# jscanvic/Scale-Equivariant-Imaging

Measured on AMD Instinct MI355X. Metric: training images/sec (256x256 crops), proposed-loss deblur, higher is better.
Workload: dtype bf16; 1 GPU; BASELINE configs[1]: deblurring Gaussian_R2 noise=5, proposed loss (SURE + scale-EI), 256x256 pairs cropped to 48 in Loss.forward, ConvolutionalModel hidden=32 scales=5; parameters=645063043, batch_per_gpu=32, global_batch=32, parallelism=dp1

## Files before the change

### include/sei_hip.h

```cpp
#ifndef SEI_HIP_H
#define SEI_HIP_H

#include <stddef.h>
#include <stdint.h>

#ifdef __cplusplus
extern "C" {
#endif

#define SEI_OK 0
#define SEI_ERR_BAD_ARG 10001
#define SEI_ERR_TOO_LARGE 10002


#define SEI_ABI_VERSION 12
int sei_abi_version(void);
int sei_build_target(char *name, int n);

int sei_event_create(void **event);
int sei_event_destroy(void *event);
int sei_event_record_external(void *event, void *stream);
int sei_stream_wait_event(void *stream, void *event);

int sei_graph_node_counts(void *graph, int *kernel_nodes, int *all_nodes);
// ... 51 lines not shown
int sei_conv3x3_bwd_weight(const float *x, const float *gy, float *gw, float *gb, int B, int H, int W,
                           int Cin, int Cout, int nchw_x, int nchw_gy, void *stream);
size_t sei_conv3x3_bwd_weight_parts_count(int B, int H, int W, int Cin, int Cout, int nchw_x, int nchw_gy);
int sei_conv3x3_bwd_weight_parts(const float *x, const float *gy, float *part, int B, int H, int W, int Cin, int Cout,
                                 int nchw_x, int nchw_gy, void *stream);

int sei_dwconv7_fwd(const float *x, const float *w, const float *bias, const float *res,
                    float res_scale, float *y, int B, int H, int W, int C, int flip, void *stream);
size_t sei_dwconv7_bwd_weight_workspace(int B, int H, int W, int C);
int sei_dwconv7_bwd_weight(const float *x, const float *gy, float *gw, float *gbias, int B, int H,
                           int W, int C, float *work, size_t work_floats, void *stream);
int sei_dwconv7_fwd_ex(const float *x, const float *w, const float *bias, const float *res,
                       float res_scale, float *y, int B, int H, int W, int C, int flip, int seg, void *stream);
size_t sei_dwconv7_bwd_weight_workspace_ex(int B, int H, int W, int C, int seg);
int sei_dwconv7_bwd_weight_ex(const float *x, const float *gy, float *gw, float *gbias, int B, int H,
                              int W, int C, float *work, size_t work_floats, int seg, void *stream);
int sei_dwconv7_ln_fwd(const float *x, const float *w, const float *bias, const float *gamma, const float *beta,
                       float *h1, void *h2, int out16, float *mean, float *rstd, int B, int H, int W, int C,
                       float eps, void *stream);
int sei_dwconv7_ln_fwd_ex(const float *x, const float *w, const float *bias, const float *gamma, const float *beta,
                          float *h1, void *h2, int out16, float *mean, float *rstd, int B, int H, int W, int C,
                          float eps, int fuse, void *stream);
size_t sei_dwconv7_ln_fwd_launches(int B, int H, int W, int C);

int sei_ln_fwd(const float *x, const float *gamma, const float *beta, float *y, float *mean,
               float *rstd, size_t rows, int C, float eps, void *stream);
size_t sei_ln_bwd_workspace(size_t rows, int C);
size_t sei_ln_bwd_part_offset(size_t rows, int C);
size_t sei_ln_bwd_part_count(size_t rows, int C);
int sei_ln_bwd(const float *x, const float *gamma, const float *mean, const float *rstd,
               const float *gy, float *gx, float *ggamma, float *gbeta, size_t rows, int C,
               float *work, size_t work_floats, void *stream);
int sei_ln_bwd_res(const float *x, const float *gamma, const float *mean, const float *rstd,
                   const float *gy, const float *res, float *gx, float *ggamma, float *gbeta, size_t rows, int C,
                   float *work, size_t work_floats, void *stream);

#define SEI_FOLD_SPLIT 0
#define SEI_FOLD_DWCONV7 1
#define SEI_FOLD_MAX_JOBS 48
typedef struct SeiFoldJob {
    float *a, *b, *c;
    int ncol, split, kind, nseg;
    const float *part[3];
    int groups[3];
    int reserved;
} SeiFoldJob;
// ... 229 lines not shown
```

### scale-equivariant-imaging_amd/_native.py

```python
import ctypes
import os

import torch

_HERE = os.path.dirname(os.path.abspath(__file__))
LIB_PATH = os.environ.get("SEI_HIP_LIBRARY") or os.path.join(_HERE, "libsei_hip.so")

SEI_REDUCE_BLOCKS = 256

_c = ctypes
_P, _I, _F, _Z, _L = _c.c_void_p, _c.c_int, _c.c_float, _c.c_size_t, _c.c_longlong

SIGNATURES = {
    "sei_abi_version": [],
    "sei_event_create": [_P],
    "sei_event_destroy": [_P],
    "sei_event_record_external": [_P, _P],
    "sei_stream_wait_event": [_P, _P],
    "sei_graph_node_counts": [_P, _P, _P],
    "sei_build_target": [_c.c_char_p, _I],
    "sei_blur_sep_circ": [_P, _P, _P, _P, _I, _I, _I, _I, _I, _I, _P],
    "sei_blur_dense_circ": [_P, _P, _P, _I, _I, _I, _I, _I, _I, _P],
    "sei_resample_sepband": [_P, _P, _I, _I, _I, _I, _I, _P, _P, _I, _I, _P, _P, _I, _I, _P],
    "sei_scale_params": [_P, _P, _P, _I, _I, _P, _P, _P],
# ... 4 lines not shown
    "sei_axpy": [_P, _P, _F, _P, _Z, _P],
    "sei_stack_axpy": [_P, _P, _F, _P, _Z, _P],
    "sei_proposed_draws": [_c.c_ulonglong, _c.c_ulonglong, _P, _I, _I, _I, _I, _I, _P, _I, _P, _P, _P, _P],
    "sei_crop_window": [_P, _P, _I, _I, _I, _I, _I, _I, _P],
    "sei_concat2_f32": [_P, _Z, _P, _Z, _P, _P],
    "sei_scale_dev_f32": [_P, _P, _P, _Z, _P],
    "sei_add_scalars": [_P, _P, _P, _P],
    "sei_zero_ranges": [_P, _P, _I, _P],
    "sei_sure_terms": [_P, _P, _P, _P, _I, _I, _I, _I, _I, _F, _F, _F, _P, _P, _P, _P, _P],
    "sei_mse_terms": [_P, _P, _Z, _F, _P, _P, _P, _P],
    "sei_sure_loss": [_P, _P, _P, _P, _I, _I, _I, _I, _I, _F, _F, _F, _F, _P, _P, _P, _P, _P],
    "sei_mse_loss": [_P, _P, _Z, _F, _F, _P, _P, _P, _P],
    "sei_luma_sqerr": [_P, _P, _Z, _P, _P, _P],
    "sei_ssim_luma": [_P, _P, _I, _I, _I, _P, _P, _P],
    "sei_conv3x3_fwd": [_P, _P, _P, _P, _P, _I, _I, _I, _I, _I, _I, _I, _I, _P],
    "sei_conv3x3_bwd_weight": [_P, _P, _P, _P, _I, _I, _I, _I, _I, _I, _I, _P],
    "sei_conv3x3_bwd_weight_parts": [_P, _P, _P, _I, _I, _I, _I, _I, _I, _I, _P],
    "sei_dwconv7_fwd": [_P, _P, _P, _P, _F, _P, _I, _I, _I, _I, _I, _P],
    "sei_dwconv7_bwd_weight": [_P, _P, _P, _P, _I, _I, _I, _I, _P, _Z, _P],
    "sei_dwconv7_fwd_ex": [_P, _P, _P, _P, _F, _P, _I, _I, _I, _I, _I, _I, _P],
    "sei_dwconv7_bwd_weight_ex": [_P, _P, _P, _P, _I, _I, _I, _I, _P, _Z, _I, _P],
    "sei_dwconv7_ln_fwd": [_P, _P, _P, _P, _P, _P, _P, _I, _P, _P, _I, _I, _I, _I, _F, _P],
    "sei_dwconv7_ln_fwd_ex": [_P, _P, _P, _P, _P, _P, _P, _I, _P, _P, _I, _I, _I, _I, _F, _I, _P],
    "sei_ln_fwd": [_P, _P, _P, _P, _P, _P, _Z, _I, _F, _P],
    "sei_ln_bwd": [_P, _P, _P, _P, _P, _P, _P, _P, _Z, _I, _P, _Z, _P],
    "sei_ln_bwd_res": [_P, _P, _P, _P, _P, _P, _P, _P, _P, _Z, _I, _P, _Z, _P],
    "sei_gemm_f32": [_P, _P, _P, _I, _I, _I, _I, _I, _I, _P, _P, _P, _P, _P],
    "sei_gemm_f32_ex": [_P, _P, _P, _I, _I, _I, _I, _I, _I, _P, _P, _P, _P, _I, _L, _L, _L, _I, _P],
    "sei_gemm_bf16_ex": [_P, _P, _P, _I, _I, _I, _I, _I, _I, _P, _P, _P, _P, _I, _L, _L, _L, _I, _P],
    "sei_gemm_bf16_mixed": [_P, _I, _P, _I, _P, _I, _I, _I, _I, _I, _I, _P, _P, _P, _P, _I, _L, _L, _L, _I, _P],
    "sei_cast_bf16": [_P, _P, _Z, _P],
    "sei_weight_shadow_bf16": [_P, _P, _P, _I, _I, _P],
    "sei_ln_fwd_bf16": [_P, _P, _P, _P, _P, _P, _Z, _I, _F, _P],
    "sei_colsum_bf16": [_P, _P, _Z, _I, _P],
    "sei_split_bf16x2": [_P, _P, _Z, _P],
    "sei_split_bf16x3": [_P, _P, _Z, _I, _P],
    "sei_gelu_f32": [_P, _P, _Z, _P],
    "sei_mul_dgelu_f32": [_P, _P, _Z, _P],
    "sei_cast_transpose_bf16": [_P, _I, _P, _P, _I, _I, _I, _P, _P],
    "sei_cast_bf16_colsum_weighted": [_P, _P, _P, _P, _I, _I, _P],
    "sei_cast_bf16_colsum_parts": [_P, _P, _P, _P, _I, _I, _P],
    "sei_gemm_bf16nt": [_P, _I, _I, _P, _I, _I, _P, _P, _I, _I, _I, _I, _P, _P, _P, _P, _P],
    "sei_gemm_bf16nt_colsum": [_P, _I, _I, _P, _I, _I, _P, _I, _I, _I, _I, _P, _P, _P],
    "sei_gemm_bf16nt_ws": [_P, _I, _I, _P, _I, _I, _P, _P, _I, _I, _I, _I, _P, _P, _P, _P, _P, _P, _Z, _I, _I, _I, _P],
    "sei_fold_many": [_P, _I, _P],
    "sei_transpose_bf16_many": [_P, _I, _P],
# ... 64 lines not shown
DWSTREAM_MAX_JOBS = 64


class FoldJob(_c.Structure):
    _fields_ = [("a", _P), ("b", _P), ("c", _P), ("ncol", _I), ("split", _I), ("kind", _I), ("nseg", _I),
                ("part", _P * 3), ("groups", _I * 3), ("reserved", _I)]


FOLD_SPLIT, FOLD_DWCONV7, FOLD_MAX_JOBS = 0, 1, 48


class TransposeJob(_c.Structure):
    _fields_ = [("src", _P), ("dst", _P), ("R", _I), ("C", _I)]


TRANSPOSE_MAX_JOBS = 16


SIZE_QUERIES = {
    "sei_proposed_draws_max_numel": [],
    "sei_ssim_luma_work_floats": [_I, _I, _I],
    "sei_dwconv7_bwd_weight_workspace": [_I, _I, _I, _I],
    "sei_dwconv7_bwd_weight_workspace_ex": [_I, _I, _I, _I, _I],
    "sei_ln_bwd_workspace": [_Z, _I],
    "sei_dwconv7_ln_fwd_launches": [_I, _I, _I, _I],
    "sei_sepmap2_bf16_eligible": [_I, _I, _I, _I, _I, _I],
    "sei_sepmap2_bf16_pack_elems": [_I, _I, _I, _I],
    "sei_sepmap2_big_eligible": [_I, _I, _I, _I, _I, _I],
    "sei_sepmap2_big_pack_elems": [_I, _I, _I, _I],
    "sei_sepmap2_big_work_elems": [_I, _I, _I, _I, _I, _I],
    "sei_swin_partials_floats": [_I],
    "sei_tokgrad_bf16_eligible": [_I, _I, _I, _I, _L, _L],
    "sei_dwstream_bf16_eligible": [_I, _I, _I, _I, _L, _L],
    "sei_mlp_fused_eligible": [_L, _I],
    "sei_rowgemm_bf16_eligible": [_L, _I, _I, _I, _I],
    "sei_rowgemm_lnbwd_bf16_eligible": [_L, _I, _I],
    "sei_rowgemm_lnbwd_work_floats": [_I],
    "sei_ln_bwd_part_offset": [_Z, _I],
    "sei_ln_bwd_part_count": [_Z, _I],
    "sei_rowgemm_dgelu_bf16_eligible": [_L, _I, _I],
    "sei_rowgemm_ln_bf16_eligible": [_L, _I, _I],
    "sei_gemm_bf16nt_plan": [_I, _I, _I, _I, _I, _I, _I, _I],
    "sei_gemm_bf16nt_plan_ws": [_I, _I, _I, _I, _I, _I, _I, _I, _Z],
    "sei_conv3x3_bwd_weight_parts_count": [_I, _I, _I, _I, _I, _I, _I],
    "sei_sepmap2_small_eligible": [_I, _I, _I, _I, _I, _I],
    "sei_cast_bf16_colsum_parts_count": [_I, _I],
# ... 152 lines not shown
```

### scale-equivariant-imaging_amd/models/_ops.py

```python
import os

import torch

import _native as N
from . import _mats

EPI_NONE, EPI_BIAS, EPI_BIAS_GELU, EPI_BIAS_RES, EPI_MUL_DGELU, EPI_ACCUM, EPI_BIAS_ROWSCALE = range(7)
LN_EPS = 1e-6


def grad_of(p):
    if p.grad is None:
        view = getattr(p, "_sei_grad_view", None)
        if view is None or view.shape != p.shape or view.device != p.device:
            view = torch.zeros_like(p, memory_format=torch.contiguous_format)
        else:
            view.zero_()
        p.grad = view
    return p.grad


_ARENA = None


# ... 347 lines not shown
    M = B * H * W
    h1 = _alloc((B, H, W, C), torch.float32, x.device)
    h2 = _alloc((M, C), torch.bfloat16 if out16 else torch.float32, x.device)
    mean = _alloc((M,), torch.float32, x.device)
    rstd = _alloc((M,), torch.float32, x.device)
    args = (x.data_ptr(), w.data_ptr(), N.ptr(bias), gamma.data_ptr(), beta.data_ptr(), h1.data_ptr(), h2.data_ptr(),
            int(out16), mean.data_ptr(), rstd.data_ptr(), B, H, W, C, LN_EPS)
    if fuse:
        N.call("sei_dwconv7_ln_fwd_ex", *args, int(fuse))
    else:
        N.call("sei_dwconv7_ln_fwd", *args)
    return h1, h2, mean, rstd


def dwconv7_weight_grad(x, gy, gw, gb, seg=0):
    B, H, W, C = x.shape
    need = N.lib().sei_dwconv7_bwd_weight_workspace_ex(B, H, W, C, int(seg))
    work = torch.empty(need, dtype=torch.float32, device=x.device)
    deferred = need > 0 and defer_fold(gw, gb, None, 50 * C, C, N.FOLD_DWCONV7, work, 0, need // (50 * C))
    leaf_call(gw, "sei_dwconv7_bwd_weight_ex", x.data_ptr(), gy.data_ptr(), None if deferred else gw.data_ptr(),
              None if deferred else N.ptr(gb), B, H, W, C, work.data_ptr(), need, int(seg), keep=(x, gy, work))


def sepmap2(x, mats, Ho, Wo):
    B, Hi, Wi, C = x.shape
    y = _alloc((B, Ho, Wo, C), torch.float32, x.device)
    work = torch.empty(2 * B * Hi * Wo * C, dtype=torch.float32, device=x.device)
    RW, LH = (mats[4], mats[5]) if len(mats) >= 6 else _mats.pack_for_kernel(mats[:4], x.device)
    N.call("sei_sepmap2_packed", x.data_ptr(), y.data_ptr(), B, Hi, Wi, Ho, Wo, C, RW.data_ptr(), LH.data_ptr(),
           work.data_ptr(), work.numel())
    return y


_SEPMAP_MFMA = __import__("os").environ.get("SEI_SEPMAP_F32") != "1"
_SEPMAP_SMALL = __import__("os").environ.get("SEI_NO_SEPMAP_SMALL") != "1"


def sepmap2_16(x, mats, Ho, Wo, out16=False):
    B, Hi, Wi, C = x.shape
    if _SEPMAP_SMALL and x.is_cuda and N.lib().sei_sepmap2_small_eligible(B, Hi, Wi, Ho, Wo, C):
        y = _alloc((B, Ho, Wo, C), torch.bfloat16 if out16 else torch.float32, x.device)
        L1, R1, L2, R2 = mats[:4]
        N.call("sei_sepmap2_small", x.data_ptr(), y.data_ptr(), int(out16), B, Hi, Wi, Ho, Wo, C, L1.data_ptr(),
               R1.data_ptr(), L2.data_ptr(), R2.data_ptr())
        return y
    small = _SEPMAP_MFMA and x.is_cuda and max(Hi, Wi, Ho, Wo) <= 64 and N.lib().sei_sepmap2_bf16_eligible(B, Hi, Wi, Ho, Wo, C)
# ... 16 lines not shown


def _packed16(mats, big=False):
    L1, R1, L2, R2 = mats[:4]
    key = (L1.data_ptr(), R1.data_ptr(), L2.data_ptr(), R2.data_ptr(), tuple(L1.shape), tuple(R1.shape), big)
    hit = _PACKED16.get(key)
    if hit is None:
        (Ho, Hi), (Wo, Wi) = L1.shape, R1.shape
        kind = "sei_sepmap2_big" if big else "sei_sepmap2_bf16"
        out = torch.empty(getattr(N.lib(), kind + "_pack_elems")(Hi, Wi, Ho, Wo), dtype=torch.int16, device=L1.device)
        N.call(kind + "_pack", L1.data_ptr(), R1.data_ptr(), L2.data_ptr(), R2.data_ptr(), out.data_ptr(), Hi, Wi,
               Ho, Wo)
        hit = _PACKED16[key] = (out, L1, R1, L2, R2)
    return hit[0]


def _nhwc(x):
    N.check_tensor(x, "activation")
    if x.dim() != 4:
        raise ValueError("expected an NHWC activation (B, H, W, C)")
    return x


class ConvBlockFn(torch.autograd.Function):
    @staticmethod
    def forward(ctx, x, w1, b1, gamma, beta, w2, b2, w3, b3, twice):
        _no_joint_form()
        ctx.dtype = get_compute_dtype()
        x = _nhwc(x)
        B, H, W, C = x.shape
        M = B * H * W
        h1, h2, mean, rstd = dwconv7_ln(x, w1, b1, gamma, beta, out16=False)
        h4 = torch.empty((M, 4 * C), dtype=torch.float32, device=x.device)
        h3 = gemm(h2, w2, M, 4 * C, C, 0, 1, EPI_BIAS_GELU, bias=b2, D2=h4)
        out = gemm(h4, w3, M, C, 4 * C, 0, 1, EPI_BIAS_RES, bias=b3, R1=x, R2=x if twice else None)
        ctx.save_for_backward(x, h1, mean, rstd, h2, h3, h4)
        ctx.params = (w1, b1, gamma, beta, w2, b2, w3, b3)
        ctx.twice = twice
        return out.view(B, H, W, C)

    @_in_forward_mode
    def backward(ctx, go):
        x, h1, mean, rstd, h2, h3, h4 = ctx.saved_tensors
        w1, b1, gamma, beta, w2, b2, w3, b3 = ctx.params
        B, H, W, C = x.shape
        M = B * H * W
        go = go.contiguous()
        go2 = go.view(M, C)
        colsum_into(grad_of(b3), go2)
        gemm(go2, h4, C, 4 * C, M, 1, 0, EPI_ACCUM, out=grad_of(w3).view(C, 4 * C))
        gh3 = gemm(go2, w3, M, 4 * C, C, 0, 0, EPI_MUL_DGELU, R1=h3)
        colsum_into(grad_of(b2), gh3)
        gemm(gh3, h2, 4 * C, C, M, 1, 0, EPI_ACCUM, out=grad_of(w2).view(4 * C, C))
        gh2 = gemm(gh3, w2, M, C, 4 * C, 0, 0, EPI_NONE)
        gh1 = layer_norm_bwd(h1.view(M, C), gamma, mean, rstd, gh2, grad_of(gamma), grad_of(beta))
        gh1 = gh1.view(B, H, W, C)
        dwconv7_weight_grad(x, gh1, grad_of(w1), grad_of(b1))
        gx = None
        if ctx.needs_input_grad[0]:
            gx = dwconv7(gh1, w1, None, flip=True, res=go, res_scale=2.0 if ctx.twice else 1.0)
        return (gx,) + (None,) * 9


class DownsampleFn(torch.autograd.Function):

    @staticmethod
    def forward(ctx, x, gamma, beta, w, b, rate, with_skip=False):
        _no_joint_form()
        ctx.dtype = get_compute_dtype()
        ctx.set_materialize_grads(False)
        x = _nhwc(x)
        B, H, W, C = x.shape
        M, Co = B * H * W, w.shape[0]
        h, mean, rstd = layer_norm(x.view(M, C), gamma, beta)
        fwd, bwd = _mats.resample_matrices("down", H, W, rate, x.device)
        Ho, Wo = fwd[0].shape[0], fwd[1].shape[0]
        u = sepmap2(h.view(B, H, W, C), fwd, Ho, Wo)
        Mo = B * Ho * Wo
        s = _mats.constant_response("down", H, W, rate, x.device, B)
        out = gemm(u.view(Mo, C), w, Mo, Co, C, 0, 1, EPI_BIAS_ROWSCALE, bias=b, R1=s)
        ctx.save_for_backward(x, mean, rstd, u, s)
        ctx.params, ctx.mats_t, ctx.hw = (gamma, beta, w, b), bwd, (H, W, Ho, Wo)
        out = out.view(B, Ho, Wo, Co)
        return (out, x) if with_skip else out
# ... 156 lines not shown
    M, Nn = x16.shape
    if leaf:
        leaf_call(acc, "sei_colsum_bf16", x16.data_ptr(), acc.data_ptr(), M, Nn, keep=(x16,))
    else:
        N.call("sei_colsum_bf16", x16.data_ptr(), acc.data_ptr(), M, Nn)


def colsum16_into_inline(acc, x16):
    colsum16_into(acc, x16, leaf=False)


def gemm_mixed(A, Bm, M, Nn, K, ta, tb, epi, out=None, bias=None, R1=None, R2=None, D2=None, allow_splitk=True):
    if out is None:
        out = torch.empty((M, Nn), dtype=torch.float32, device=A.device)
    _gemm_call(2.0 * M * Nn * K, "sei_gemm_bf16_mixed", A.data_ptr(), int(A.dtype == torch.bfloat16), Bm.data_ptr(),
               int(Bm.dtype == torch.bfloat16), out.data_ptr(), M, Nn, K, ta, tb, epi, N.ptr(bias), N.ptr(R1),
               N.ptr(R2), N.ptr(D2), 1, 0, 0, 0, int(allow_splitk))
    return out


CAST_COLSUM_PARTS = os.environ.get("SEI_CAST_COLSUM_ATOMICS") != "1"


def cast16(x2d, colsum_into_=None, row_weight=None):
    R, C = x2d.shape
    x16 = _alloc((R, C), torch.bfloat16, x2d.device)
    if colsum_into_ is not None and CAST_COLSUM_PARTS and C % 4 == 0:
        parts = N.lib().sei_cast_bf16_colsum_parts_count(R, C)
        ms = _state_for(colsum_into_.data_ptr())["milestone"]
        early = ms is not None and min(ms[0]) <= colsum_into_.data_ptr() <= max(ms[0])
        if parts > 0 and not early:
            work = torch.empty(parts * C, dtype=torch.float32, device=x2d.device)
            if defer_fold(colsum_into_, None, None, C, C, N.FOLD_SPLIT, work, 0, parts):
                N.call("sei_cast_bf16_colsum_parts", x2d.data_ptr(), x16.data_ptr(), N.ptr(row_weight), work.data_ptr(), R, C)
                return x16
    if row_weight is not None and colsum_into_ is not None and C % 4 == 0:
        N.call("sei_cast_bf16_colsum_weighted", x2d.data_ptr(), x16.data_ptr(), row_weight.data_ptr(), colsum_into_.data_ptr(),
               R, C)
        return x16
    if row_weight is not None and colsum_into_ is not None:
        colsum_into(colsum_into_, x2d, row_weight=row_weight)
        colsum_into_ = None
    N.call("sei_cast_transpose_bf16", x2d.data_ptr(), 0, x16.data_ptr(), None, R, C, R, N.ptr(colsum_into_))
    return x16


def _fresh_state():
# ... 440 lines not shown
        part = stale[k:k + N.TRANSPOSE_MAX_JOBS]
        outs = [torch.empty((q16.shape[1], q16.shape[0]), dtype=torch.bfloat16, device=q16.device) for _, q16, _ in part]
        jobs = (N.TransposeJob * len(part))(*[N.TransposeJob(q16.data_ptr(), o.data_ptr(), q16.shape[0], q16.shape[1])
                                             for (_, q16, _), o in zip(part, outs)])
        N.call("sei_transpose_bf16_many", jobs, len(part))
        for (q, _, qkey), o in zip(part, outs):
            q._sei_shadow_t = (qkey, o, capturing)
    return p._sei_shadow_t[1]


def _transposed16(w16):
    R, C = w16.shape
    wt = torch.empty((C, R), dtype=torch.bfloat16, device=w16.device)
    N.call("sei_cast_transpose_bf16", w16.data_ptr(), 1, None, wt.data_ptr(), R, C, R, None)
    return wt


class ConvBlockFn16(torch.autograd.Function):

    @staticmethod
    def forward(ctx, x, w1, b1, gamma, beta, w2, b2, w3, b3, twice):
        ctx.dtype = get_compute_dtype()
        x = _nhwc(x)
        B, H, W, C = x.shape
        M = B * H * W
        h1, h2, mean, rstd = dwconv7_ln(x, w1, b1, gamma, beta, out16=True)
        w2_16, w3_16 = shadow(w2), shadow(w3)
        ctx.fused = fused_mlp_ok(M, C)
        _tape(ConvBlockFn16, ctx)
        if ctx.fused:
            out = _alloc((M, C), torch.float32, x.device)
            N.call("sei_mlp_fused_fwd", h2.data_ptr(), w2_16.data_ptr(), b2.data_ptr(), w3_16.data_ptr(), b3.data_ptr(),
                   x.data_ptr(), 2.0 if twice else 1.0, out.data_ptr(), M, C)
            if _GEMM_PROFILE is not None:
                _GEMM_PROFILE.append((4.0 * M * 4 * C * C, "sei_mlp_fused_fwd",
                                      (h2.data_ptr(), w2_16.data_ptr(), b2.data_ptr(), w3_16.data_ptr(), b3.data_ptr(),
                                       x.data_ptr(), 2.0 if twice else 1.0, out.data_ptr(), M, C)))
            ctx.save_for_backward(x, h1, mean, rstd, h2)
            ctx.params = (w1, b1, gamma, beta, w2, b2, w3, b3)
            ctx.twice = twice
            return out.view(B, H, W, C)
        h3 = _alloc((M, 4 * C), torch.float32, x.device)
        h4 = _alloc((M, 4 * C), torch.bfloat16, x.device)
        gemm_nt16(h2, w2_16, M, 4 * C, C, EPI_BIAS_GELU, out32=h3, bias=b2, D2_16=h4)
        out = _alloc((M, C), torch.float32, x.device)
        gemm_nt16(h4, w3_16, M, C, 4 * C, EPI_BIAS_RES, out32=out, bias=b3, R1=x, R2=x if twice else None)
        ctx.save_for_backward(x, h1, mean, rstd, h2, h3, h4)
        ctx.params = (w1, b1, gamma, beta, w2, b2, w3, b3)
        ctx.twice = twice
        return out.view(B, H, W, C)

    @_in_forward_mode
    def backward(ctx, go):
        if ctx.fused:
            return ConvBlockFn16._backward_fused(ctx, go)
        x, h1, mean, rstd, h2, h3, h4 = ctx.saved_tensors
        w1, b1, gamma, beta, w2, b2, w3, b3 = ctx.params
        B, H, W, C = x.shape
        M = B * H * W
        go = go.contiguous()
        go2 = go.view(M, C)
        go16 = cast16(go2, colsum_into_=grad_of(b3))
        gh3 = torch.empty((M, 4 * C), dtype=torch.bfloat16, device=x.device)
        gemm_nt16(go16, shadow(w3), M, 4 * C, C, EPI_MUL_DGELU, out16=gh3, R1=h3, b_rmajor=True, colsum=grad_of(b2))
        weight_grad16(go16, h4, grad_of(w3).view(C, 4 * C))
        gh2 = torch.empty((M, C), dtype=torch.float32, device=x.device)
        gemm_nt16(gh3, shadow(w2), M, C, 4 * C, EPI_NONE, out32=gh2, b_rmajor=True)
        weight_grad16(gh3, h2, grad_of(w2).view(4 * C, C))
        gh1 = layer_norm_bwd(h1.view(M, C), gamma, mean, rstd, gh2, grad_of(gamma), grad_of(beta)).view(B, H, W, C)
        dwconv7_weight_grad(x, gh1, grad_of(w1), grad_of(b1))
        gx = None
        if ctx.needs_input_grad[0]:
            gx = dwconv7(gh1, w1, None, flip=True, res=go, res_scale=2.0 if ctx.twice else 1.0)
        return (gx,) + (None,) * 9


    @staticmethod
    def _backward_fused(ctx, go):
        x, h1, mean, rstd, h2 = ctx.saved_tensors
        w1, b1, gamma, beta, w2, b2, w3, b3 = ctx.params
        B, H, W, C = x.shape
        M = B * H * W
        go = go.contiguous()
        dev = x.device
        w2_16, w3_16 = shadow(w2), shadow(w3)
        gh2 = torch.empty((M, C), dtype=torch.float32, device=dev)
        go16 = torch.empty((M, C), dtype=torch.bfloat16, device=dev)
        h4 = torch.empty((M, 4 * C), dtype=torch.bfloat16, device=dev)
        gh3 = torch.empty((M, 4 * C), dtype=torch.bfloat16, device=dev)
        w3t, w2t = _transposed16_cached(w3, w3_16), _transposed16_cached(w2, w2_16)
        args = (go.data_ptr(), h2.data_ptr(), w2_16.data_ptr(), b2.data_ptr(), w3t.data_ptr(), w2t.data_ptr(),
                gh2.data_ptr(), go16.data_ptr(), h4.data_ptr(), gh3.data_ptr(), M, C)
        N.call("sei_mlp_fused_bwd", *args)
        if _GEMM_PROFILE is not None:
            _GEMM_PROFILE.append((4.0 * M * 4 * C * C, "sei_mlp_fused_bwd", args))
        if DWSTREAM and N.lib().sei_dwstream_bf16_eligible(C, 4 * C, C, 4 * C, M, 0):
            weight_grad16(go16, h4, grad_of(w3).view(C, 4 * C), bias=grad_of(b3))
            weight_grad16(gh3, h2, grad_of(w2).view(4 * C, C), bias=grad_of(b2))
        else:
            colsum_into(grad_of(b3), go.view(M, C))
            colsum16_into(grad_of(b2), gh3)
            weight_grad16(go16, h4, grad_of(w3).view(C, 4 * C))
            weight_grad16(gh3, h2, grad_of(w2).view(4 * C, C))
        gh1 = layer_norm_bwd(h1.view(M, C), gamma, mean, rstd, gh2, grad_of(gamma), grad_of(beta)).view(B, H, W, C)
        dwconv7_weight_grad(x, gh1, grad_of(w1), grad_of(b1))
        gx = None
        if ctx.needs_input_grad[0]:
            gx = dwconv7(gh1, w1, None, flip=True, res=go, res_scale=2.0 if ctx.twice else 1.0)
        return (gx,) + (None,) * 9


class DownsampleFn16(torch.autograd.Function):

    @staticmethod
    def forward(ctx, x, gamma, beta, w, b, rate, with_skip=False):
        ctx.dtype = get_compute_dtype()
        ctx.set_materialize_grads(False)
        x = _nhwc(x)
        B, H, W, C = x.shape
        M, Co = B * H * W, w.shape[0]
        h, mean, rstd = layer_norm(x.view(M, C), gamma, beta)
        fwd, bwd = _mats.resample_matrices("down", H, W, rate, x.device)
        Ho, Wo = fwd[0].shape[0], fwd[1].shape[0]
        u = sepmap2_16(h.view(B, H, W, C), fwd, Ho, Wo, out16=True)
        Mo = B * Ho * Wo
        s = _mats.constant_response("down", H, W, rate, x.device, B)
        u16 = u.view(Mo, C) if u.dtype == torch.bfloat16 else cast16(u.view(Mo, C))
        out = _alloc((Mo, Co), torch.float32, x.device)
        gemm_nt16(u16, shadow(w), Mo, Co, C, EPI_BIAS_ROWSCALE, out32=out, bias=b, R1=s)
        ctx.save_for_backward(x, mean, rstd, u16, s)
        ctx.params, ctx.mats_t, ctx.hw = (gamma, beta, w, b), bwd, (H, W, Ho, Wo)
        ctx.with_skip, ctx.rate = with_skip, rate
        _tape(DownsampleFn16, ctx)
        out = out.view(B, Ho, Wo, Co)
        return (out, x) if with_skip else out

    @_in_forward_mode
    def backward(ctx, go, gskip=None):
        x, mean, rstd, u16, s = ctx.saved_tensors
        gamma, beta, w, b = ctx.params
        B, H, W, C = x.shape
        Ho, Wo = ctx.hw[2], ctx.hw[3]
        M, Mo, Co = B * H * W, B * Ho * Wo, w.shape[0]
        go2 = go.contiguous().view(Mo, Co)
        go16 = cast16(go2, colsum_into_=grad_of(b), row_weight=s)
        gu = torch.empty((Mo, C), dtype=torch.float32, device=x.device)
        gemm_nt16(go16, shadow(w), Mo, C, Co, EPI_NONE, out32=gu, b_rmajor=True)
        weight_grad16(go16, u16, grad_of(w).view(Co, C))
        gh = sepmap2_16(gu.view(B, Ho, Wo, C), ctx.mats_t, H, W).view(M, C)
        res = None if gskip is None else gskip.contiguous().view(M, C)
        gx = layer_norm_bwd(x.view(M, C), gamma, mean, rstd, gh, grad_of(gamma), grad_of(beta), res=res).view(B, H, W, C)
        return (gx if ctx.needs_input_grad[0] else None), None, None, None, None, None, None


class UpsampleFn16(torch.autograd.Function):
    @staticmethod
    def forward(ctx, x, skip, gamma, beta, w, b, rate):
        ctx.dtype = get_compute_dtype()
        x = _nhwc(x)
        B, H, W, C = x.shape
        Co = w.shape[0]
        fwd, bwd = _mats.resample_matrices("up", H, W, rate, x.device)
        Ho, Wo = fwd[0].shape[0], fwd[1].shape[0]
        u = sepmap2_16(x, fwd, Ho, Wo)
        M = B * Ho * Wo
        h, mean, rstd = layer_norm16(u.view(M, C), gamma, beta)
        w16 = shadow(w)
        out = _alloc((M, Co), torch.float32, x.device)
        _tape(UpsampleFn16, ctx)
        if skip is not None:
            skip = _nhwc(skip)
            if tuple(skip.shape) != (B, Ho, Wo, Co):
                raise ValueError("skip connection shape mismatch")
            gemm_nt16(h, w16, M, Co, C, EPI_BIAS_RES, out32=out, bias=b, R1=skip)
        else:
            gemm_nt16(h, w16, M, Co, C, EPI_BIAS, out32=out, bias=b)
        ctx.save_for_backward(u, mean, rstd, h)
        ctx.params, ctx.mats_t, ctx.in_hw = (gamma, beta, w, b), bwd, (H, W)
        return out.view(B, Ho, Wo, Co)

    @_in_forward_mode
    def backward(ctx, go):
        u, mean, rstd, h = ctx.saved_tensors
        gamma, beta, w, b = ctx.params
        B, Ho, Wo, C = u.shape
        M, Co = B * Ho * Wo, w.shape[0]
        go = go.contiguous()
        go2 = go.view(M, Co)
        go16 = cast16(go2, colsum_into_=grad_of(b))
        gh = torch.empty((M, C), dtype=torch.float32, device=u.device)
        gemm_nt16(go16, shadow(w), M, C, Co, EPI_NONE, out32=gh, b_rmajor=True)
        weight_grad16(go16, h, grad_of(w).view(Co, C))
        gu = layer_norm_bwd(u.view(M, C), gamma, mean, rstd, gh, grad_of(gamma), grad_of(beta))
        gx = None
        if ctx.needs_input_grad[0]:
            gx = sepmap2_16(gu.view(B, Ho, Wo, C), ctx.mats_t, *ctx.in_hw)
        gskip = go if ctx.needs_input_grad[1] else None
        return gx, gskip, None, None, None, None, None


class Conv3x3Fn(torch.autograd.Function):
    @staticmethod
    def forward(ctx, x, w, b, res, nchw_in, nchw_out):
        N.check_tensor(x, "conv3x3 input")
        Co, Ci = w.shape[0], w.shape[1]
        if nchw_in:
            B, _, H, W = x.shape
        else:
            B, H, W, _ = x.shape
        y = _alloc((B, Co, H, W) if nchw_out else (B, H, W, Co), torch.float32, x.device)
        _tape(Conv3x3Fn, ctx)
        if res is not None:
# ... 88 lines not shown
```

Before: 2721 images/s.

## Fuse depthwise 7x7 conv backward input and weight gradients into one tiled kernel

Adds a HIP kernel that computes the depthwise 7x7 input gradient and weight/bias gradient in one pass over a shared LDS tile of the output gradient. Global-to-LDS loads are double-buffered. The same kernel can also emit a bf16 copy of the input gradient plus partial column sums, so the next Down/Upsample backward can skip its separate cast16 and colsum pass. This removes repeated reads of gy and x and extra launches per ConvBlock backward, at the cost of a large, register-heavy kernel with one workgroup per CU and more complex fold and side-channel bookkeeping.

Result: no change. 2720 images/s, median of 2 (-0.1%).

```diff
diff --git a/include/sei_hip.h b/include/sei_hip.h
--- a/include/sei_hip.h
+++ b/include/sei_hip.h
@@ -97,6 +97,11 @@
                           float *h1, void *h2, int out16, float *mean, float *rstd, int B, int H, int W, int C,
                           float eps, int fuse, void *stream);
 size_t sei_dwconv7_ln_fwd_launches(int B, int H, int W, int C);
+size_t sei_dwconv7_bwd_pair_workspace(int B, int H, int W, int C);
+size_t sei_dwconv7_bwd_pair_colparts(int B, int H, int W, int C);
+int sei_dwconv7_bwd_pair(const float *x, const float *gy, const float *w, const float *res, float res_scale,
+                         float *gx, uint16_t *gx16, const float *row_weight, float *colpart, float *work,
+                         size_t work_floats, int B, int H, int W, int C, void *stream);
 
 int sei_ln_fwd(const float *x, const float *gamma, const float *beta, float *y, float *mean,
                float *rstd, size_t rows, int C, float eps, void *stream);
diff --git a/scale-equivariant-imaging_amd/_native.py b/scale-equivariant-imaging_amd/_native.py
--- a/scale-equivariant-imaging_amd/_native.py
+++ b/scale-equivariant-imaging_amd/_native.py
@@ -50,6 +50,7 @@
     "sei_dwconv7_bwd_weight_ex": [_P, _P, _P, _P, _I, _I, _I, _I, _P, _Z, _I, _P],
     "sei_dwconv7_ln_fwd": [_P, _P, _P, _P, _P, _P, _P, _I, _P, _P, _I, _I, _I, _I, _F, _P],
     "sei_dwconv7_ln_fwd_ex": [_P, _P, _P, _P, _P, _P, _P, _I, _P, _P, _I, _I, _I, _I, _F, _I, _P],
+    "sei_dwconv7_bwd_pair": [_P, _P, _P, _P, _F, _P, _P, _P, _P, _P, _Z, _I, _I, _I, _I, _P],
     "sei_ln_fwd": [_P, _P, _P, _P, _P, _P, _Z, _I, _F, _P],
     "sei_ln_bwd": [_P, _P, _P, _P, _P, _P, _P, _P, _Z, _I, _P, _Z, _P],
     "sei_ln_bwd_res": [_P, _P, _P, _P, _P, _P, _P, _P, _P, _Z, _I, _P, _Z, _P],
@@ -160,6 +161,8 @@
     "sei_ssim_luma_work_floats": [_I, _I, _I],
     "sei_dwconv7_bwd_weight_workspace": [_I, _I, _I, _I],
     "sei_dwconv7_bwd_weight_workspace_ex": [_I, _I, _I, _I, _I],
+    "sei_dwconv7_bwd_pair_workspace": [_I, _I, _I, _I],
+    "sei_dwconv7_bwd_pair_colparts": [_I, _I, _I, _I],
     "sei_ln_bwd_workspace": [_Z, _I],
     "sei_dwconv7_ln_fwd_launches": [_I, _I, _I, _I],
     "sei_sepmap2_bf16_eligible": [_I, _I, _I, _I, _I, _I],
diff --git a/scale-equivariant-imaging_amd/csrc/dwconv_pair.hip b/scale-equivariant-imaging_amd/csrc/dwconv_pair.hip
--- /dev/null
+++ b/scale-equivariant-imaging_amd/csrc/dwconv_pair.hip
@@ -0,0 +1,375 @@
+#include "sei_common.h"
+
+namespace {
+
+typedef __attribute__((address_space(3))) void lds_void;
+typedef __attribute__((address_space(1))) const void glb_void;
+
+__device__ __attribute__((aligned(16))) float g_pr_zero_chunk[4] = {0.f, 0.f, 0.f, 0.f};
+
+constexpr int PR_THREADS = 256;
+constexpr int PR_CC = 32;
+constexpr int PR_ROWS = PR_THREADS / PR_CC;
+constexpr int PR_MAXK = 10;
+constexpr int PR_WBYTES = PR_CC * 49 * 4;
+constexpr int PR_WPIECES = 7;
+constexpr int PR_SUMS = 52;
+
+__device__ __forceinline__ unsigned short pr_f2bf(float v) {
+    const __bf16 b = (__bf16)v;
+    return __builtin_bit_cast(unsigned short, b);
+}
+
+__device__ __forceinline__ void pr_csum(float &cs, float &comp, float w, float v, bool weighted) {
+    const float p = weighted ? w * v : v;
+    const float y = p - (weighted ? comp - fmaf(w, v, -p) : comp);
+    const float t = cs + y;
+    comp = (t - cs) - y;
+    cs = t;
+}
+
+__device__ __forceinline__ void pr_wait_vmcnt(int n) {
+    switch (n) {
+#define SEI_PR_W(N_) case N_: asm volatile("s_waitcnt vmcnt(" #N_ ")" ::: "memory"); break;
+        SEI_PR_W(1) SEI_PR_W(2) SEI_PR_W(3) SEI_PR_W(4) SEI_PR_W(5) SEI_PR_W(6) SEI_PR_W(7) SEI_PR_W(8)
+        SEI_PR_W(9) SEI_PR_W(10) SEI_PR_W(11) SEI_PR_W(12) SEI_PR_W(13) SEI_PR_W(14) SEI_PR_W(15) SEI_PR_W(16)
+#undef SEI_PR_W
+        default: asm volatile("s_waitcnt vmcnt(0)" ::: "memory"); break;
+    }
+}
+
+constexpr int pr_pieces(int tw) { return ((PR_ROWS + 6) * (tw + 6) + 7) / 8; }
+constexpr int pr_lds_bytes(int tw) { return 2 * pr_pieces(tw) * 1024; }
+static_assert(pr_lds_bytes(12) >= PR_ROWS * PR_SUMS * PR_CC * 4 && pr_pieces(12) * 1024 >= PR_WPIECES * 1024,
+              "the tile buffers also hold the weights (prologue) and the reduction of the sums (epilogue)");
+static_assert(pr_lds_bytes(16) <= 160 * 1024, "one workgroup per CU");
+
+template <int TW>
+__global__ __launch_bounds__(PR_THREADS, 1) void dwconv7_pair_tiled_kernel(
+    const float *__restrict__ x, const float *__restrict__ gy, const float *__restrict__ w,
+    const float *__restrict__ res, float res_scale, float *__restrict__ gx, unsigned short *__restrict__ gx16,
+    const float *__restrict__ row_weight, float *__restrict__ colpart, float *__restrict__ part, int H, int W, int C,
+    int th, int tiles_i, int tiles_j, int ntiles, int tiles_per_block, int npix, int npieces) {
+    constexpr int tw = TW, lw = TW + 6, tile_bytes = pr_pieces(TW) * 1024;
+    __shared__ __attribute__((aligned(16))) char smem[pr_lds_bytes(TW)];
+    const int lane = threadIdx.x & 63, wave = __builtin_amdgcn_readfirstlane(threadIdx.x >> 6);
+    const int cl = threadIdx.x & (PR_CC - 1), tr = threadIdx.x >> 5;
+    const int g = blockIdx.y, c0 = g * PR_CC;
+    const int s0 = blockIdx.x * tiles_per_block, s1 = min(ntiles, s0 + tiles_per_block);
+
+    int pp[PR_MAXK];
+#pragma unroll
+    for (int k = 0; k < PR_MAXK; ++k) {
+        const int pixel = 8 * (wave + 4 * k) + (lane >> 3);
+        const int lr = pixel / lw;
+        pp[k] = pixel < npix ? (lr << 8) | (pixel - lr * lw) : -1;
+    }
+    struct Tile {
+        int b, i0, j0;
+    };
+    auto decode = [&](int s) {
+        Tile t;
+        const int tj = s % tiles_j, rest = s / tiles_j;
+        const int ti = rest % tiles_i;
+        t.b = rest / tiles_i;
+        t.i0 = ti * th;
+        t.j0 = tj * tw;
+        return t;
+    };
+    auto issue_tile = [&](const Tile &t, char *dst) {
+        const float *gb = gy + (size_t)t.b * H * W * C + c0 + 4 * (lane & 7);
+#pragma unroll
+        for (int k = 0; k < PR_MAXK; ++k) {
+            const int q = wave + 4 * k;
+            if (q < npieces) {
+                const int lr = pp[k] >> 8, lc = pp[k] & 255;
+                const int ii = t.i0 - 3 + lr, jj = t.j0 - 3 + lc;
+                const bool ok = pp[k] >= 0 && ii >= 0 && ii < H && jj >= 0 && jj < W;
+                const float *src = ok ? gb + ((size_t)ii * W + jj) * C : g_pr_zero_chunk;
+                __builtin_amdgcn_global_load_lds((glb_void *)src, (lds_void *)(dst + q * 1024), 16, 0, 0);
+            }
+        }
+    };
+    char *const tile0 = smem;
+
+    Tile cur = decode(s0);
+    issue_tile(cur, tile0);
+    {
+        const char *wsrc = reinterpret_cast<const char *>(w + (size_t)c0 * 49);
+#pragma unroll
+        for (int k = 0; k < 2; ++k) {
+            const int p = wave + 4 * k;
+            if (p < PR_WPIECES) {
+                const int off = 1024 * p + 16 * lane;
+                const char *src = off < PR_WBYTES ? wsrc + off : reinterpret_cast<const char *>(g_pr_zero_chunk);
+                __builtin_amdgcn_global_load_lds((glb_void *)src, (lds_void *)(smem + tile_bytes + p * 1024), 16, 0, 0);
+            }
+        }
+    }
+    asm volatile("s_waitcnt vmcnt(0)" ::: "memory");
+    __syncthreads();
+    float wr[49];
+    {
+        const float *wl = reinterpret_cast<const float *>(smem + tile_bytes);
+#pragma unroll
+        for (int t = 0; t < 49; ++t) wr[t] = wl[cl * 49 + 48 - t];
+    }
+    __syncthreads();
+
+    float acc[49];
+#pragma unroll
+    for (int t = 0; t < 49; ++t) acc[t] = 0.f;
+    float acc_b = 0.f, cs = 0.f, cs_comp = 0.f;
+
+    int later = 0;
+    for (int s = s0; s < s1; ++s) {
+        const int par = (s - s0) & 1;
+        const char *tile = tile0 + par * tile_bytes;
+        pr_wait_vmcnt(later);
+        __builtin_amdgcn_s_barrier();
+        asm volatile("" ::: "memory");
+        const int i = cur.i0 + tr;
+        const bool row_ok = tr < th && i < H;
+        const int jn = min(tw, W - cur.j0);
+        const size_t pix0 = ((size_t)cur.b * H + i) * W + cur.j0;
+        const size_t obase = pix0 * C + c0 + cl;
+        float gv[TW], xv[TW];
+        float rw_own = 1.f;
+        if (row_ok) {
+#pragma unroll
+            for (int jl = 0; jl < TW; ++jl) xv[jl] = (jl < jn) ? x[obase + (size_t)jl * C] : 0.f;
+            if (res) {
+#pragma unroll
+                for (int jl = 0; jl < TW; ++jl) gv[jl] = (jl < jn) ? res[obase + (size_t)jl * C] : 0.f;
+            }
+            if (row_weight && cl < jn) rw_own = row_weight[pix0 + cl];
+        }
+        asm volatile("" ::: "memory");
+        Tile nxt = cur;
+        if (s + 1 < s1) {
+            nxt = decode(s + 1);
+            issue_tile(nxt, tile0 + (par ^ 1) * tile_bytes);
+        }
+        asm volatile("" ::: "memory");
+        {
+            const int r0 = 2 * wave;
+            later = (r0 < th && cur.i0 + r0 < H) ? jn : 0;
+        }
+        if (row_ok) {
+            const float *trow = reinterpret_cast<const float *>(tile) + (tr * lw) * PR_CC + cl;
+            constexpr int rs_ = lw * PR_CC;
+            constexpr int RW = 10;
+            const int hw = lane & 32;
+            float ring[7][RW];
+#pragma unroll
+            for (int c = 0; c < 6; ++c)
+#pragma unroll
+                for (int di = 0; di < 7; ++di) ring[di][c % RW] = trow[di * rs_ + c * PR_CC];
+#pragma unroll
+            for (int blk = 0; blk < TW / 4; ++blk) {
+#pragma unroll
+                for (int c = 4 * blk + 6; c < 4 * blk + 10; ++c)
+#pragma unroll
+                    for (int di = 0; di < 7; ++di) ring[di][c % RW] = trow[di * rs_ + c * PR_CC];
+                float a[4] = {0.f, 0.f, 0.f, 0.f};
+#pragma unroll
+                for (int di = 0; di < 7; ++di)
+#pragma unroll
+                    for (int dj = 0; dj < 7; ++dj)
+#pragma unroll
+                        for (int o = 0; o < 4; ++o) {
+                            const float v = ring[di][(4 * blk + o + dj) % RW];
+                            a[o] = fmaf(wr[di * 7 + dj], v, a[o]);
+                            acc[di * 7 + dj] = fmaf(xv[4 * blk + o], v, acc[di * 7 + dj]);
+                        }
+#pragma unroll
+                for (int o = 0; o < 4; ++o) {
+                    const int jl = 4 * blk + o;
+                    if (res) a[o] = fmaf(res_scale, gv[jl], a[o]);
+                    const float rwv = row_weight ? __shfl(rw_own, hw + jl, 64) : 1.f;
+                    if (jl < jn) {
+                        gx[obase + (size_t)jl * C] = a[o];
+                        if (gx16) gx16[obase + (size_t)jl * C] = pr_f2bf(a[o]);
+                        acc_b += ring[3][(jl + 3) % RW];
+                        pr_csum(cs, cs_comp, rwv, a[o], row_weight != nullptr);
+                    }
+                }
+            }
+        }
+        cur = nxt;
+    }
+
+    __syncthreads();
+    float *red = reinterpret_cast<float *>(smem);
+#pragma unroll
+    for (int t = 0; t < 49; ++t) red[(tr * PR_SUMS + 48 - t) * PR_CC + cl] = acc[t];
+    red[(tr * PR_SUMS + 49) * PR_CC + cl] = acc_b;
+    red[(tr * PR_SUMS + 50) * PR_CC + cl] = cs;
+    red[(tr * PR_SUMS + 51) * PR_CC + cl] = cs_comp;
+    __syncthreads();
+    float *out = part + (size_t)blockIdx.x * 50 * C + c0;
+    for (int e = threadIdx.x; e < 51 * PR_CC; e += PR_THREADS) {
+        const int t = e >> 5, c2 = e & 31;
+        if (t < 50) {
+            float sum = 0.f;
+#pragma unroll
+            for (int r = 0; r < PR_ROWS; ++r) sum += red[(r * PR_SUMS + t) * PR_CC + c2];
+            out[(size_t)t * C + c2] = sum;
+        } else if (colpart) {
+            double sum = 0.0;
+#pragma unroll
+            for (int r = 0; r < PR_ROWS; ++r)
+                sum += (double)red[(r * PR_SUMS + 50) * PR_CC + c2] - (double)red[(r * PR_SUMS + 51) * PR_CC + c2];
+            colpart[(size_t)blockIdx.x * C + c0 + c2] = (float)sum;
+        }
+    }
+}
+
+template <int S>
+__global__ __launch_bounds__(PR_THREADS) void dwconv7_pair_whole_kernel(
+    const float *__restrict__ x, const float *__restrict__ gy, const float *__restrict__ w,
+    const float *__restrict__ res, float res_scale, float *__restrict__ gx, unsigned short *__restrict__ gx16,
+    const float *__restrict__ row_weight, float *__restrict__ colpart, float *__restrict__ part, int B, int C,
+    int imgs_per_thread) {
+    __shared__ float wl[PR_THREADS * 49];
+    const int c0 = blockIdx.x * PR_THREADS, c = c0 + threadIdx.x;
+    {
+        const int nw = min(PR_THREADS, C - c0) * 49;
+        for (int e = threadIdx.x; e < nw; e += PR_THREADS) wl[e] = w[(size_t)c0 * 49 + e];
+        __syncthreads();
+    }
+    if (c >= C) return;
+    const int b0 = blockIdx.y * imgs_per_thread, b1 = min(B, b0 + imgs_per_thread);
+    constexpr int LO = (S >= 4) ? 0 : 4 - S, HI = 6 - LO;
+    float wr[49], acc[49];
+#pragma unroll
+    for (int t = 0; t < 49; ++t) {
+        const int di = t / 7, dj = t % 7;
+        const bool used = di >= LO && di <= HI && dj >= LO && dj <= HI;
+        wr[t] = used ? wl[threadIdx.x * 49 + 48 - t] : 0.f;
+        acc[t] = 0.f;
+    }
+    float acc_b = 0.f, cs = 0.f, cs_comp = 0.f;
+    for (int b = b0; b < b1; ++b) {
+        const size_t base = (size_t)b * S * S * C + c;
+        float gi[S][S], xi[S][S];
+#pragma unroll
+        for (int i = 0; i < S; ++i)
+#pragma unroll
+            for (int j = 0; j < S; ++j) {
+                gi[i][j] = gy[base + (size_t)(i * S + j) * C];
+                xi[i][j] = x[base + (size_t)(i * S + j) * C];
+                acc_b += gi[i][j];
+            }
+#pragma unroll
+        for (int i = 0; i < S; ++i)
+#pragma unroll
+            for (int j = 0; j < S; ++j) {
+                float a = 0.f;
+#pragma unroll
+                for (int di = 0; di < 7; ++di)
+#pragma unroll
+                    for (int dj = 0; dj < 7; ++dj) {
+                        const int ii = i + di - 3, jj = j + dj - 3;
+                        if (ii >= 0 && ii < S && jj >= 0 && jj < S) {
+                            a = fmaf(wr[di * 7 + dj], gi[ii][jj], a);
+                            acc[di * 7 + dj] = fmaf(xi[i][j], gi[ii][jj], acc[di * 7 + dj]);
+                        }
+                    }
+                const size_t o = base + (size_t)(i * S + j) * C;
+                if (res) a = fmaf(res_scale, res[o], a);
+                gx[o] = a;
+                if (gx16) gx16[o] = pr_f2bf(a);
+                pr_csum(cs, cs_comp, row_weight ? row_weight[(size_t)b * S * S + i * S + j] : 1.f, a, row_weight != nullptr);
+            }
+    }
+    float *out = part + (size_t)blockIdx.y * 50 * C + c;
+#pragma unroll
+    for (int t = 0; t < 49; ++t) out[(size_t)(48 - t) * C] = acc[t];
+    out[(size_t)49 * C] = acc_b;
+    if (colpart) colpart[(size_t)blockIdx.y * C + c] = cs - cs_comp;
+}
+
+struct PrPlan {
+    int kind;
+    int th, tw, tiles_i, tiles_j, ntiles, tpb, npix, npieces, ipt;
+    unsigned gx, gy;
+    size_t nparts;
+};
+
+inline PrPlan pr_plan(int B, int H, int W, int C) {
+    PrPlan p{};
+    if (B <= 0 || H <= 0 || W <= 0 || C <= 0 || C % PR_CC != 0) return p;
+    if ((size_t)B * H * W * C >= ((size_t)1 << 40)) return p;
+    if ((H == 3 && W == 3) || (H == 6 && W == 6)) {
+        p.gx = (unsigned)sei_ceil_div(C, PR_THREADS);
+        size_t want = (size_t)B * H * W / 64;
+        if (want < 8) want = 8;
+        if (want * p.gx < 256) want = sei_ceil_div(256, p.gx);
+        if (want > (size_t)B) want = B;
+        p.ipt = (int)sei_ceil_div(B, want);
+        p.gy = (unsigned)sei_ceil_div(B, p.ipt);
+        if (p.gy > 65535) return p;
+        p.nparts = p.gy;
+        p.kind = H;
+        return p;
+    }
+    if (H < 8 || W < 8) return p;
+    const int G = C / PR_CC;
+    if (G > 65535) return p;
+    p.th = (H % 8 == 0) ? 8 : ((H % 6 == 0) ? 6 : ((H % 7 == 0) ? 7 : 8));
+    p.tw = (W % 12 == 0) ? 12 : 16;
+    p.tiles_i = (int)sei_ceil_div(H, p.th);
+    p.tiles_j = (int)sei_ceil_div(W, p.tw);
+    const size_t nt = (size_t)B * p.tiles_i * p.tiles_j;
+    if (nt >= ((size_t)1 << 30)) return p;
+    p.ntiles = (int)nt;
+    p.npix = (p.th + 6) * (p.tw + 6);
+    p.npieces = (p.npix + 7) / 8;
+    size_t want = 256 / (size_t)G;
+    if (want < 8) want = 8;
+    p.tpb = (int)sei_ceil_div(nt, want);
+    p.gx = (unsigned)sei_ceil_div(nt, (size_t)p.tpb);
+    p.gy = (unsigned)G;
+    p.nparts = p.gx;
+    p.kind = 1;
+    return p;
+}
+
+}
+
+extern "C" size_t sei_dwconv7_bwd_pair_workspace(int B, int H, int W, int C) {
+    return pr_plan(B, H, W, C).nparts * 50 * (size_t)(C > 0 ? C : 0);
+}
+
+extern "C" size_t sei_dwconv7_bwd_pair_colparts(int B, int H, int W, int C) { return pr_plan(B, H, W, C).nparts; }
+
+extern "C" int sei_dwconv7_bwd_pair(const float *x, const float *gy, const float *w, const float *res, float res_scale,
+                                    float *gx, uint16_t *gx16, const float *row_weight, float *colpart, float *work,
+                                    size_t work_floats, int B, int H, int W, int C, void *stream) {
+    SEI_REQUIRE(x && gy && w && gx && work && gx != gy && gx != x && (colpart || !row_weight));
+    const PrPlan p = pr_plan(B, H, W, C);
+    SEI_REQUIRE(p.kind != 0 && work_floats >= p.nparts * 50 * (size_t)C);
+    SEI_REQUIRE(((reinterpret_cast<uintptr_t>(gy) | reinterpret_cast<uintptr_t>(w)) & 15) == 0);
+    SEI_REQUIRE(((reinterpret_cast<uintptr_t>(x) | reinterpret_cast<uintptr_t>(res) | reinterpret_cast<uintptr_t>(gx) |
+                  reinterpret_cast<uintptr_t>(row_weight) | reinterpret_cast<uintptr_t>(colpart) |
+                  reinterpret_cast<uintptr_t>(work)) & 3) == 0 && (reinterpret_cast<uintptr_t>(gx16) & 1) == 0);
+    hipStream_t s = (hipStream_t)stream;
+    unsigned short *g16 = gx16;
+    if (p.kind == 1) {
+#define SEI_PR_TILED(TW_)                                                                                              \
+    hipLaunchKernelGGL((dwconv7_pair_tiled_kernel<TW_>), dim3(p.gx, p.gy), dim3(PR_THREADS), 0, s, x, gy, w, res,      \
+                       res_scale, gx, g16, row_weight, colpart, work, H, W, C, p.th, p.tiles_i, p.tiles_j, p.ntiles,   \
+                       p.tpb, p.npix, p.npieces)
+        if (p.tw == 12) SEI_PR_TILED(12);
+        else SEI_PR_TILED(16);
+#undef SEI_PR_TILED
+    } else if (p.kind == 3) {
+        hipLaunchKernelGGL((dwconv7_pair_whole_kernel<3>), dim3(p.gx, p.gy), dim3(PR_THREADS), 0, s, x, gy, w, res,
+                           res_scale, gx, g16, row_weight, colpart, work, B, C, p.ipt);
+    } else {
+        hipLaunchKernelGGL((dwconv7_pair_whole_kernel<6>), dim3(p.gx, p.gy), dim3(PR_THREADS), 0, s, x, gy, w, res,
+                           res_scale, gx, g16, row_weight, colpart, work, B, C, p.ipt);
+    }
+    return sei_launch_status();
+}
diff --git a/scale-equivariant-imaging_amd/models/_ops.py b/scale-equivariant-imaging_amd/models/_ops.py
--- a/scale-equivariant-imaging_amd/models/_ops.py
+++ b/scale-equivariant-imaging_amd/models/_ops.py
@@ -393,6 +393,63 @@
               None if deferred else N.ptr(gb), B, H, W, C, work.data_ptr(), need, int(seg), keep=(x, gy, work))
 
 
+DW_PAIR = os.environ.get("SEI_NO_DW_PAIR") != "1"
+DW_PAIR_MIN_EXTENT = int(os.environ.get("SEI_DW_PAIR_MIN_EXTENT", "16"))
+
+
+def _fold_now(a, b, ncol, split, kind, work, groups):
+    job = N.FoldJob()
+    job.a, job.b, job.c, job.ncol, job.split, job.kind, job.nseg = a.data_ptr(), N.ptr(b), None, ncol, split, kind, 1
+    job.part[0], job.groups[0] = work.data_ptr(), groups
+    N.call("sei_fold_many", (N.FoldJob * 1)(job), 1)
+
+
+def wants_grad16(out, resampler=()):
+    out._sei_grad16 = tuple(resampler)
+    return out
+
+
+def dwconv7_bwd_pair(x, gh1, w1, gw, gb, go, res_scale, grad16=None):
+    B, H, W, C = x.shape
+    if not (DW_PAIR and not LEAF_STREAM and x.is_cuda and N.aligned(gh1, w1) and min(H, W) >= DW_PAIR_MIN_EXTENT):
+        return None
+    need = N.lib().sei_dwconv7_bwd_pair_workspace(B, H, W, C)
+    if need == 0:
+        return None
+    groups = need // (50 * C)
+    work = torch.empty(need, dtype=torch.float32, device=x.device)
+    if not defer_fold(gw, gb, None, 50 * C, C, N.FOLD_DWCONV7, work, 0, groups):
+        return None
+    gx = torch.empty_like(x)
+    gx16 = colpart = rw = None
+    if grad16 is not None:
+        gx16 = torch.empty((B * H * W, C), dtype=torch.bfloat16, device=x.device)
+        colpart = torch.empty(groups * C, dtype=torch.float32, device=x.device)
+        if grad16:
+            rw = _mats.constant_response(*grad16, x.device, B)
+    N.call("sei_dwconv7_bwd_pair", x.data_ptr(), gh1.data_ptr(), w1.data_ptr(), go.data_ptr(), float(res_scale),
+           gx.data_ptr(), N.ptr(gx16), N.ptr(rw), N.ptr(colpart), work.data_ptr(), need, B, H, W, C)
+    if gx16 is not None:
+        gx._sei_cast16 = (gx.data_ptr(), gx._version, gx16, colpart, groups, N.ptr(rw))
+    return gx
+
+
+def _cast16_from_producer(src, x2d, colsum_into_, row_weight):
+    side = getattr(src, "_sei_cast16", None)
+    if side is None:
+        return None
+    ptr, version, x16, colpart, groups, rw_ptr = side
+    R, C = x2d.shape
+    if ptr != x2d.data_ptr() or version != src._version or tuple(x16.shape) != (R, C) or rw_ptr != N.ptr(row_weight):
+        return None
+    if colsum_into_ is not None:
+        ms = _state_for(colsum_into_.data_ptr())["milestone"]
+        early = ms is not None and min(ms[0]) <= colsum_into_.data_ptr() <= max(ms[0])
+        if early or not defer_fold(colsum_into_, None, None, C, C, N.FOLD_SPLIT, colpart, 0, groups):
+            _fold_now(colsum_into_, None, C, C, N.FOLD_SPLIT, colpart, groups)
+    return x16
+
+
 def sepmap2(x, mats, Ho, Wo):
     B, Hi, Wi, C = x.shape
     y = _alloc((B, Ho, Wo, C), torch.float32, x.device)
@@ -455,6 +512,18 @@
     return x
 
 
+def _convblock_tail(ctx, x, gh1, w1, b1, go):
+    scale = 2.0 if ctx.twice else 1.0
+    if ctx.needs_input_grad[0]:
+        gx = dwconv7_bwd_pair(x, gh1, w1, grad_of(w1), grad_of(b1), go, scale, getattr(ctx, "grad16", None))
+        if gx is not None:
+            return gx
+    dwconv7_weight_grad(x, gh1, grad_of(w1), grad_of(b1))
+    if ctx.needs_input_grad[0]:
+        return dwconv7(gh1, w1, None, flip=True, res=go, res_scale=scale)
+    return None
+
+
 class ConvBlockFn(torch.autograd.Function):
     @staticmethod
     def forward(ctx, x, w1, b1, gamma, beta, w2, b2, w3, b3, twice):
@@ -488,11 +557,7 @@
         gh2 = gemm(gh3, w2, M, C, 4 * C, 0, 0, EPI_NONE)
         gh1 = layer_norm_bwd(h1.view(M, C), gamma, mean, rstd, gh2, grad_of(gamma), grad_of(beta))
         gh1 = gh1.view(B, H, W, C)
-        dwconv7_weight_grad(x, gh1, grad_of(w1), grad_of(b1))
-        gx = None
-        if ctx.needs_input_grad[0]:
-            gx = dwconv7(gh1, w1, None, flip=True, res=go, res_scale=2.0 if ctx.twice else 1.0)
-        return (gx,) + (None,) * 9
+        return (_convblock_tail(ctx, x, gh1, w1, b1, go),) + (None,) * 9
 
 
 class DownsampleFn(torch.autograd.Function):
@@ -695,7 +760,11 @@
 CAST_COLSUM_PARTS = os.environ.get("SEI_CAST_COLSUM_ATOMICS") != "1"
 
 
-def cast16(x2d, colsum_into_=None, row_weight=None):
+def cast16(x2d, colsum_into_=None, row_weight=None, src=None):
+    if src is not None:
+        hit = _cast16_from_producer(src, x2d, colsum_into_, row_weight)
+        if hit is not None:
+            return hit
     R, C = x2d.shape
     x16 = _alloc((R, C), torch.bfloat16, x2d.device)
     if colsum_into_ is not None and CAST_COLSUM_PARTS and C % 4 == 0:
@@ -1182,6 +1251,7 @@
     def forward(ctx, x, w1, b1, gamma, beta, w2, b2, w3, b3, twice):
         ctx.dtype = get_compute_dtype()
         x = _nhwc(x)
+        ctx.grad16 = getattr(x, "_sei_grad16", None)
         B, H, W, C = x.shape
         M = B * H * W
         h1, h2, mean, rstd = dwconv7_ln(x, w1, b1, gamma, beta, out16=True)
@@ -1228,11 +1298,7 @@
         gemm_nt16(gh3, shadow(w2), M, C, 4 * C, EPI_NONE, out32=gh2, b_rmajor=True)
         weight_grad16(gh3, h2, grad_of(w2).view(4 * C, C))
         gh1 = layer_norm_bwd(h1.view(M, C), gamma, mean, rstd, gh2, grad_of(gamma), grad_of(beta)).view(B, H, W, C)
-        dwconv7_weight_grad(x, gh1, grad_of(w1), grad_of(b1))
-        gx = None
-        if ctx.needs_input_grad[0]:
-            gx = dwconv7(gh1, w1, None, flip=True, res=go, res_scale=2.0 if ctx.twice else 1.0)
-        return (gx,) + (None,) * 9
+        return (_convblock_tail(ctx, x, gh1, w1, b1, go),) + (None,) * 9
 
 
     @staticmethod
@@ -1263,11 +1329,7 @@
             weight_grad16(go16, h4, grad_of(w3).view(C, 4 * C))
             weight_grad16(gh3, h2, grad_of(w2).view(4 * C, C))
         gh1 = layer_norm_bwd(h1.view(M, C), gamma, mean, rstd, gh2, grad_of(gamma), grad_of(beta)).view(B, H, W, C)
-        dwconv7_weight_grad(x, gh1, grad_of(w1), grad_of(b1))
-        gx = None
-        if ctx.needs_input_grad[0]:
-            gx = dwconv7(gh1, w1, None, flip=True, res=go, res_scale=2.0 if ctx.twice else 1.0)
-        return (gx,) + (None,) * 9
+        return (_convblock_tail(ctx, x, gh1, w1, b1, go),) + (None,) * 9
 
 
 class DownsampleFn16(torch.autograd.Function):
@@ -1292,7 +1354,7 @@
         ctx.params, ctx.mats_t, ctx.hw = (gamma, beta, w, b), bwd, (H, W, Ho, Wo)
         ctx.with_skip, ctx.rate = with_skip, rate
         _tape(DownsampleFn16, ctx)
-        out = out.view(B, Ho, Wo, Co)
+        out = wants_grad16(out.view(B, Ho, Wo, Co), ("down", H, W, rate))
         return (out, x) if with_skip else out
 
     @_in_forward_mode
@@ -1302,8 +1364,9 @@
         B, H, W, C = x.shape
         Ho, Wo = ctx.hw[2], ctx.hw[3]
         M, Mo, Co = B * H * W, B * Ho * Wo, w.shape[0]
-        go2 = go.contiguous().view(Mo, Co)
-        go16 = cast16(go2, colsum_into_=grad_of(b), row_weight=s)
+        go = go.contiguous()
+        go2 = go.view(Mo, Co)
+        go16 = cast16(go2, colsum_into_=grad_of(b), row_weight=s, src=go)
         gu = torch.empty((Mo, C), dtype=torch.float32, device=x.device)
         gemm_nt16(go16, shadow(w), Mo, C, Co, EPI_NONE, out32=gu, b_rmajor=True)
         weight_grad16(go16, u16, grad_of(w).view(Co, C))
@@ -1337,7 +1400,7 @@
             gemm_nt16(h, w16, M, Co, C, EPI_BIAS, out32=out, bias=b)
         ctx.save_for_backward(u, mean, rstd, h)
         ctx.params, ctx.mats_t, ctx.in_hw = (gamma, beta, w, b), bwd, (H, W)
-        return out.view(B, Ho, Wo, Co)
+        return wants_grad16(out.view(B, Ho, Wo, Co))
 
     @_in_forward_mode
     def backward(ctx, go):
@@ -1347,7 +1410,7 @@
         M, Co = B * Ho * Wo, w.shape[0]
         go = go.contiguous()
         go2 = go.view(M, Co)
-        go16 = cast16(go2, colsum_into_=grad_of(b))
+        go16 = cast16(go2, colsum_into_=grad_of(b), src=go)
         gh = torch.empty((M, C), dtype=torch.float32, device=u.device)
         gemm_nt16(go16, shadow(w), M, C, Co, EPI_NONE, out32=gh, b_rmajor=True)
         weight_grad16(go16, h, grad_of(w).view(Co, C))
```
